# johndpope/SPEAK-hack

Hardware: AMD Instinct MI355X
Metric: generator frames/sec at 256^2, batch 8/GPU (higher is better)
Workload: dtype f32; 1 GPU; StyleGAN decoder (styleganv1.StyleGenerator) 256^2 forward only, batch 8/GPU, fp32, random-init weights, synthetic [8,6144] latents, device-drawn noise; global_batch=8, resolution=256, parallelism=replicas x1 (no data-path collective), launch=hipGraph replay of the step

## Files before the change

### speak-hack_amd/csrc/conv3x3_wino_f32.hip

```cpp
#include "conv_mfma_f32.hpp"

namespace spkwino {

using spkconv::f32x16;
using spkconv::lds_f32_t;
using spkconv::static_for;
typedef float f32x2 __attribute__((ext_vector_type(2)));
typedef float f32x4 __attribute__((ext_vector_type(4)));
typedef __attribute__((address_space(3))) f32x2 lds_f32x2_t;
typedef __attribute__((address_space(3))) f32x2 __attribute__((aligned(4))) lds_f32x2u_t;

constexpr int CO_T = 64, CI_T = 8, NTILE = 64, NT = 256;
constexpr int WIDE = 0, SQUARE = 1;
constexpr int region_w(int shape) { return shape == SQUARE ? 16 : 32; }
constexpr int region_h(int shape) { return shape == SQUARE ? 16 : 8; }
constexpr int RAW_PLANE = 352, RAW_WAVE = 2 * RAW_PLANE;
constexpr int RAW_GATHERS = RAW_WAVE / 64;
constexpr int U_FLOATS = 16 * CI_T * CO_T, V_FLOATS = 16 * CI_T * NTILE, RAW_FLOATS = 4 * RAW_WAVE;
constexpr int U_OFF = 0, V_OFF = 2 * U_FLOATS, RAW_OFF = V_OFF + 2 * V_FLOATS;
constexpr int PRM_OFF = RAW_OFF + 2 * RAW_FLOATS;
constexpr int DEM_OFF = PRM_OFF + 4 * CO_T;
constexpr int RGBW_OFF = DEM_OFF + CO_T;
constexpr int LDS_FLOATS = RGBW_OFF + 3 * CO_T;
constexpr int LDS_BYTES = LDS_FLOATS * 4;
// ... 48 lines not shown
    long long r = idx / CO_T;
    const int ci_l = (int)(r % CI_T);
    r /= CI_T;
    const int xi = (int)(r % 16);
    r /= 16;
    const int chunk = (int)(r % n_chunks), co_tile = (int)(r / n_chunks);
    const int co = co_tile * CO_T + co_l, ci = chunk * CI_T + ci_l;
    float v = 0.f;
    if (co < opCout && ci < opCin) {
        float g[3][3];
#pragma unroll
        for (int a = 0; a < 3; ++a)
#pragma unroll
            for (int b = 0; b < 3; ++b)
                g[a][b] = transpose_flip ? w[(((size_t)ci * Cin + co) * 3 + (2 - a)) * 3 + (2 - b)] : w[(((size_t)co * Cin + ci) * 3 + a) * 3 + b];
        const int i = xi >> 2, j = xi & 3;
        float t[3];
#pragma unroll
        for (int b = 0; b < 3; ++b)
            t[b] = i == 0 ? g[0][b] : (i == 3 ? g[2][b] : 0.5f * ((g[0][b] + g[2][b]) + (i == 1 ? g[1][b] : -g[1][b])));
        v = j == 0 ? t[0] : (j == 3 ? t[2] : 0.5f * ((t[0] + t[2]) + (j == 1 ? t[1] : -t[1])));
    }
    out[idx] = v;
}

struct PackWinoList {
    const float* w[SPK_WINO_PACK_MAX];
    float* out[SPK_WINO_PACK_MAX];
    int Cin[SPK_WINO_PACK_MAX], Cout[SPK_WINO_PACK_MAX], tf[SPK_WINO_PACK_MAX];
};

__global__ void pack_wino_list_kernel(const PackWinoList a) {
    const int it = blockIdx.y;
    const float* __restrict__ w = a.w[it];
    float* __restrict__ out = a.out[it];
    const int Cin = a.Cin[it], Cout = a.Cout[it], transpose_flip = a.tf[it];
    const int opCin = transpose_flip ? Cout : Cin, opCout = transpose_flip ? Cin : Cout;
    const int n_chunks = (opCin + CI_T - 1) / CI_T;
    const long long total = (long long)((opCout + CO_T - 1) / CO_T) * n_chunks * U_FLOATS;
    for (long long idx = (long long)blockIdx.x * blockDim.x + threadIdx.x; idx < total; idx += (long long)gridDim.x * blockDim.x) {
        const int co_l = (int)(idx % CO_T);
        long long r = idx / CO_T;
        const int ci_l = (int)(r % CI_T);
        r /= CI_T;
        const int xi = (int)(r % 16);
        r /= 16;
        const int chunk = (int)(r % n_chunks), co_tile = (int)(r / n_chunks);
        const int co = co_tile * CO_T + co_l, ci = chunk * CI_T + ci_l;
        float v = 0.f;
        if (co < opCout && ci < opCin) {
            float g[3][3];
#pragma unroll
            for (int p = 0; p < 3; ++p)
#pragma unroll
                for (int q = 0; q < 3; ++q)
                    g[p][q] = transpose_flip ? w[(((size_t)ci * Cin + co) * 3 + (2 - p)) * 3 + (2 - q)] : w[(((size_t)co * Cin + ci) * 3 + p) * 3 + q];
            const int i = xi >> 2, j = xi & 3;
            float t[3];
#pragma unroll
            for (int q = 0; q < 3; ++q)
                t[q] = i == 0 ? g[0][q] : (i == 3 ? g[2][q] : 0.5f * ((g[0][q] + g[2][q]) + (i == 1 ? g[1][q] : -g[1][q])));
            v = j == 0 ? t[0] : (j == 3 ? t[2] : 0.5f * ((t[0] + t[2]) + (j == 1 ? t[1] : -t[1])));
        }
        out[idx] = v;
    }
}

__device__ __forceinline__ float fadd_(float a, float b) { float r; asm("v_add_f32 %0, %1, %2" : "=v"(r) : "v"(a), "v"(b)); return r; }
__device__ __forceinline__ float fsub_(float a, float b) { float r; asm("v_sub_f32 %0, %1, %2" : "=v"(r) : "v"(a), "v"(b)); return r; }

__device__ __forceinline__ void up1d_(float a, float b, float c, float nkl, float nkr, float six, float& o0, float& o1, float& o2, float& o3) {
    float e, s, hl, hr;
    asm("v_sub_f32 %0, %9, %7\n\tv_add_f32 %1, %7, %9\n\tv_fma_f32 %2, %8, %12, %1\n\tv_fma_f32 %3, %8, %10, %1\n\t"
        "v_fma_f32 %4, %8, %11, %1\n\tv_fma_f32 %5, %0, -2.0, %3\n\tv_fma_f32 %6, %0, -2.0, -%4"
        : "=&v"(e), "=&v"(s), "=&v"(o1), "=&v"(hl), "=&v"(hr), "=&v"(o0), "=v"(o3)
        : "v"(a), "v"(b), "v"(c), "v"(nkl), "v"(nkr), "s"(six));
    o2 = e;
}

__device__ __forceinline__ void lds_barrier() {
    asm volatile("s_waitcnt lgkmcnt(0)\n\ts_barrier" ::: "memory");
}

template <bool MOD, int SHAPE, bool RGB = false, bool UP = false>
__global__ __launch_bounds__(NT) void wino_kernel(const Args p) {
    static_assert(!(UP && MOD), "the modulated conv keeps its x2 pass");
    constexpr int RW = region_w(SHAPE), RH = region_h(SHAPE), TXN = RW / 2, TYN = RH / 2;
    constexpr int RAW_W = UP ? RW / 2 + 2 : RW + 2, RAW_H = UP ? RH / 2 + 2 : RH + 2, RAW_USED = RAW_W * RAW_H;
    constexpr int PLANE = UP ? UP_PLANE : RAW_PLANE, NG = UP ? UP_GATHERS : RAW_GATHERS;
    extern __shared__ __attribute__((aligned(16))) float smem[];
    const int tid = threadIdx.x, lane = tid & 63;
    const int wave = __builtin_amdgcn_readfirstlane(tid >> 6);
    const int half = lane >> 5, l32 = lane & 31;
    const int wm = wave >> 1, wn = wave & 1;

    const int n_regions = p.regions_x * p.regions_y * p.B * p.ksplit;
    const int xcd = (int)blockIdx.x & 7, wk = (int)blockIdx.x >> 3, wpx = (int)gridDim.x >> 3;
    const int share_q = n_regions >> 3, share_r = n_regions & 7;
    const int reg_begin = xcd * share_q + min(xcd, share_r), reg_end = reg_begin + share_q + (xcd < share_r ? 1 : 0);
    const int grp = (int)blockIdx.y / p.co_tiles_g, co_tile = (int)blockIdx.y - grp * p.co_tiles_g, co0 = co_tile * CO_T;
    const size_t HW = (size_t)p.H * p.W;
    const int Win = UP ? p.W >> 1 : p.W;
    const size_t HWin = UP ? HW >> 2 : HW;

    const __amdgpu_buffer_rsrc_t rsrc = __builtin_amdgcn_make_buffer_rsrc(const_cast<float*>(p.x), 0, (int)p.x_bytes, 0x00020000);
    unsigned voff[NG], voff_next[NG];
    auto region_coords = [&](int item, int& b_, int& y0_, int& x0_, int& kb_) {
        const int reg = item / p.ksplit;
        kb_ = (item - reg * p.ksplit) * p.cps;
        const int rx_ = reg % p.regions_x;
        const int t_ = reg / p.regions_x;
        b_ = t_ / p.regions_y;
        y0_ = (t_ - b_ * p.regions_y) * RH;
        x0_ = rx_ * RW;
    };
    unsigned rel[NG], edge[NG];
#pragma unroll
    for (int k = 0; k < NG; ++k) {
        const int e = k * 64 + lane;
        const int j = e >= PLANE ? 1 : 0, q = e - j * PLANE;
        const int r = q / RAW_W, c = q - r * RAW_W;
        rel[k] = ((unsigned)(wave + 4 * j) * (unsigned)HWin + (unsigned)((r - 1) * Win + (c - 1))) * 4u;
        edge[k] = (r == 0 ? 1u : 0u) | (r == RAW_H - 1 ? 2u : 0u) | (c == 0 ? 4u : 0u) | (c == RAW_W - 1 ? 8u : 0u) | (q >= RAW_USED ? 16u : 0u);
    }
    auto set_voff = [&](unsigned (&vo)[NG], int b_, int y0_, int x0_) {
        const unsigned origin = (((unsigned)b_ * (unsigned)p.Cx + (unsigned)(grp * p.gin)) * (unsigned)HWin +
                                 (unsigned)(UP ? (y0_ >> 1) * Win + (x0_ >> 1) : y0_ * p.W + x0_)) * 4u;
        const unsigned at = (y0_ == 0 ? 1u : 0u) | (y0_ + RH >= p.H ? 2u : 0u) | (x0_ == 0 ? 4u : 0u) | (x0_ + RW >= p.W ? 8u : 0u) | 16u;
        if constexpr (UP) {
            const unsigned row_bytes = (unsigned)Win * 4u;
#pragma unroll
            for (int k = 0; k < NG; ++k) {
                const unsigned h = edge[k] & at;
                vo[k] = (h & 16u) ? 0x80000000u
                                  : origin + rel[k] + ((h & 1u) ? row_bytes : 0u) - ((h & 2u) ? row_bytes : 0u) + ((h & 4u) ? 4u : 0u) - ((h & 8u) ? 4u : 0u);
            }
        } else {
#pragma unroll
            for (int k = 0; k < NG; ++k) vo[k] = (edge[k] & at) ? 0x80000000u : origin + rel[k];
        }
    };
    const unsigned chunk_bytes = (unsigned)(CI_T * HWin * 4);
    const float* wsrc = p.wp + (size_t)blockIdx.y * p.n_chunks * U_FLOATS;

#define WINO_DMA_RAW(vo_in_, chunk_, slot_, k_)                                                                         \
    {                                   \
        const unsigned m0_ = (unsigned)((RAW_OFF + (slot_) * RAW_FLOATS + (k_) * 64) * 4) + raw_m0, vo_ = (vo_in_);     \
        const unsigned so_ = (unsigned)(chunk_) * chunk_bytes;                                                          \
        const __amdgpu_buffer_rsrc_t rs_ = rsrc;                                                                        \
        asm volatile("s_mov_b32 m0, %0\n\ts_nop 0\n\tbuffer_load_dword %1, %2, %3 offen lds" :: "s"(m0_), "v"(vo_), "s"(rs_), "s"(so_)); \
    }
#define WINO_DMA_U(chunk_, slot_, k_)                                                                                   \
    {                                                                                                                   \
        const unsigned m0_ = (unsigned)((U_OFF + (slot_) * U_FLOATS) * 4 + (k_) * 1024) + u_m0, vo_ = lane16;           \
        const float* sb_ = wsrc + (size_t)(chunk_) * U_FLOATS + (wave * U_DMA + (k_)) * 256;                            \
        asm volatile("s_mov_b32 m0, %0\n\ts_nop 0\n\tglobal_load_lds_dwordx4 %1, %2" :: "s"(m0_), "v"(vo_), "s"(sb_));   \
    }
#define WINO_DMA_U_BARE(chunk_, slot_, k_)                                                          \
    {                                                                                                                   \
        const unsigned m0_ = (unsigned)((U_OFF + (slot_) * U_FLOATS) * 4) + u_m0, vo_ = lane16;                         \
        const float* sb_ = wsrc + (size_t)(chunk_) * U_FLOATS + (wave * U_DMA) * 256;                                   \
        if constexpr ((k_) == 0) asm volatile("s_mov_b32 m0, %0\n\ts_nop 0" :: "s"(m0_));                               \
        asm volatile("global_load_lds_dwordx4 %0, %1" :: "v"(vo_), "s"(sb_));                                           \
    }
    const unsigned raw_m0 = (unsigned)(wave * RAW_WAVE * 4), u_m0 = (unsigned)(wave * U_DMA * 1024), lane16 = (unsigned)lane * 16u;

    int a_base = U_OFF + half * CO_T + wm * 32 + l32;
    int b_base = V_OFF + half * NTILE + wn * 32 + l32;
    const int ty_l = lane / TXN, tx_l = lane % TXN;
    int raw_rd = (RAW_OFF + wave * RAW_WAVE + 2 * ty_l * RAW_W + 2 * tx_l) >> 1;
    int v_wr = V_OFF + wave * NTILE + lane;
    asm volatile("" : "+v"(a_base), "+v"(b_base), "+v"(raw_rd), "+v"(v_wr));
    int raw_u[2][2];
    float nk[4] = {-2.f, -2.f, -2.f, -2.f}, nkn[4] = {-2.f, -2.f, -2.f, -2.f};
    const float six = 6.f;
    auto set_nk = [&](float (&k_)[4], int y0_, int x0_) {
        k_[0] = (y0_ == 0 && ty_l == 0) ? -6.f : -2.f;
        k_[1] = (y0_ + RH >= p.H && ty_l == TYN - 1) ? -6.f : -2.f;
        k_[2] = (x0_ == 0 && tx_l == 0) ? -6.f : -2.f;
        k_[3] = (x0_ + RW >= p.W && tx_l == TXN - 1) ? -6.f : -2.f;
    };
    if constexpr (UP) {
#pragma unroll
        for (int rs = 0; rs < 2; ++rs)
#pragma unroll
            for (int j = 0; j < 2; ++j) {
                raw_u[rs][j] = RAW_OFF + wave * RAW_WAVE + ty_l * RAW_W + tx_l + rs * RAW_FLOATS + j * PLANE;
                asm volatile("" : "+v"(raw_u[rs][j]));
            }
    }

    f32x16 acc[16];
    f32x16 zero16;
#pragma unroll
    for (int r = 0; r < 16; ++r) zero16[r] = 0.f;

    float d[2][16], tq[2][16], tv[2][16];
#define WINO_T_READ(rs_, j_, r_)                                                                                        \
    {                                                                                                                   \
        const f32x2 lo_ = *((const volatile lds_f32x2_t*)0 + (raw_rd + ((rs_) * RAW_FLOATS + (j_) * RAW_PLANE + (r_) * RAW_W) / 2)); \
        const f32x2 hi_ = *((const volatile lds_f32x2_t*)0 + (raw_rd + ((rs_) * RAW_FLOATS + (j_) * RAW_PLANE + (r_) * RAW_W + 2) / 2)); \
        d[j_][4 * (r_) + 0] = lo_.x; d[j_][4 * (r_) + 1] = lo_.y; d[j_][4 * (r_) + 2] = hi_.x; d[j_][4 * (r_) + 3] = hi_.y; \
    }
#define WINO_T_ROWS(j_, c_)                                                                                             \
    {                                                                                                                   \
        tq[j_][c_] = fsub_(d[j_][c_], d[j_][8 + (c_)]); tq[j_][4 + (c_)] = fadd_(d[j_][4 + (c_)], d[j_][8 + (c_)]);     \
        tq[j_][8 + (c_)] = fsub_(d[j_][8 + (c_)], d[j_][4 + (c_)]); tq[j_][12 + (c_)] = fsub_(d[j_][4 + (c_)], d[j_][12 + (c_)]); \
    }
#define WINO_T_SCALE(j_, i_, sc_)                                                                                       \
    { tv[j_][4 * (i_)] *= (sc_); tv[j_][4 * (i_) + 1] *= (sc_); tv[j_][4 * (i_) + 2] *= (sc_); tv[j_][4 * (i_) + 3] *= (sc_); }
#define WINO_T_COLS(j_, i_)                                                                                             \
    {                                                                                                                   \
        tv[j_][4 * (i_)] = fsub_(tq[j_][4 * (i_)], tq[j_][4 * (i_) + 2]); tv[j_][4 * (i_) + 1] = fadd_(tq[j_][4 * (i_) + 1], tq[j_][4 * (i_) + 2]); \
        tv[j_][4 * (i_) + 2] = fsub_(tq[j_][4 * (i_) + 2], tq[j_][4 * (i_) + 1]); tv[j_][4 * (i_) + 3] = fsub_(tq[j_][4 * (i_) + 1], tq[j_][4 * (i_) + 3]); \
    }
#define WINO_U_READ(rs_, j_, r_)                                                                                        \
    {                                                                                                                   \
        const volatile lds_f32_t* q_ = (const volatile lds_f32_t*)0 + (raw_u[rs_][j_] + (r_) * RAW_W);                  \
        const f32x2 lo_ = *reinterpret_cast<const volatile lds_f32x2u_t*>(q_);                                          \
        d[j_][3 * (r_) + 0] = lo_.x; d[j_][3 * (r_) + 1] = lo_.y; d[j_][3 * (r_) + 2] = q_[2];                          \
    }
#define WINO_U_H(j_, r_, nk_)                                                                                           \
// ... 22 lines not shown
    b_cur = b;
    kb_cur = kb;
    set_voff(voff, b, y0, x0);
    if constexpr (UP) set_nk(nk, y0, x0);
    static_for<0, U_DMA>([&](auto k) { WINO_DMA_U(kb, 0, decltype(k)::value); });
    static_for<0, NG>([&](auto k) { WINO_DMA_RAW(voff[decltype(k)::value], kb, 0, decltype(k)::value); });
    static_for<0, NG>([&](auto k) { WINO_DMA_RAW(voff[decltype(k)::value], kb + 1, 1, decltype(k)::value); });
    __builtin_amdgcn_s_waitcnt(0x0f70);
    static_for<0, 2>([&](auto j) {
        if constexpr (UP) {
            static_for<0, 3>([&](auto r) { WINO_U_READ(0, decltype(j)::value, decltype(r)::value); });
            static_for<0, 3>([&](auto r) { WINO_U_H(decltype(j)::value, decltype(r)::value, nk); });
            static_for<0, 4>([&](auto c) { WINO_U_V(decltype(j)::value, decltype(c)::value, nk); });
        } else {
            static_for<0, 4>([&](auto r) { WINO_T_READ(0, decltype(j)::value, decltype(r)::value); });
            static_for<0, 4>([&](auto c) { WINO_T_ROWS(decltype(j)::value, decltype(c)::value); });
            static_for<0, 4>([&](auto i) { WINO_T_COLS(decltype(j)::value, decltype(i)::value); });
        }
        if constexpr (MOD) {
            const float sc0_ = p.in_scale[(size_t)b * p.Cin + kb * CI_T + wave + 4 * decltype(j)::value];
            static_for<0, 4>([&](auto i) { WINO_T_SCALE(decltype(j)::value, decltype(i)::value, sc0_); });
        }
        static_for<0, 16>([&](auto xi) { WINO_T_WRITE(0, decltype(j)::value, decltype(xi)::value); });
        __builtin_amdgcn_sched_barrier(0);
    });
    __syncthreads();

#ifndef SPK_WINO_PD
#define SPK_WINO_PD 4
#endif
    constexpr int PD = SPK_WINO_PD;
    float fa[PD + 1], fb[PD + 1];
#define WINO_FRAG(slot_, s_, reg_)                                                                                      \
    {                                                                                                                   \
        constexpr int kk_ = (s_) >> 4, xi_ = (s_) & 15;                                                                 \
        fa[reg_] = *((const volatile lds_f32_t*)0 + (a_base + ((slot_) * U_FLOATS + (xi_ * CI_T + 2 * kk_) * CO_T)));   \
        fb[reg_] = *((const volatile lds_f32_t*)0 + (b_base + ((slot_) * V_FLOATS + (xi_ * CI_T + 2 * kk_) * NTILE)));  \
    }
    auto chunk_body = [&](auto slot_c, auto first_c, const int i, const float (&nk_)[4]) __attribute__((always_inline)) {
        constexpr int S = decltype(slot_c)::value, O = 1 - S;
        constexpr bool FIRST = decltype(first_c)::value;
        const int c1 = i + 1 < n ? kb_cur + i + 1 : kb;
        const int c2 = i + 2 >= n ? kb + i + 2 - n : kb_cur + i + 2;
        float msc[2] = {1.f, 1.f};
        if constexpr (MOD) {
            const float* ms_ = p.in_scale + (size_t)(i + 1 < n ? b_cur : b) * p.Cin + c1 * CI_T + wave;
            msc[0] = ms_[0];
            msc[1] = ms_[4];
        }
        static_for<0, PD>([&](auto s) { WINO_FRAG(S, decltype(s)::value, decltype(s)::value); });
        static_for<0, 64>([&](auto s_c) {
            constexpr int s = decltype(s_c)::value;
            if constexpr (s + PD < 64) { WINO_FRAG(S, s + PD, (s + PD) % (PD + 1)); }
            if constexpr (FIRST && s < 16) acc[s & 15] = __builtin_amdgcn_mfma_f32_32x32x2f32(fa[s % (PD + 1)], fb[s % (PD + 1)], zero16, 0, 0, 0);
            else acc[s & 15] = __builtin_amdgcn_mfma_f32_32x32x2f32(fa[s % (PD + 1)], fb[s % (PD + 1)], acc[s & 15], 0, 0, 0);
            if constexpr (s < U_DMA) {
                if constexpr (KO_UBARE) { WINO_DMA_U_BARE(c1, O, s); }
                else if constexpr (!KO_U) { WINO_DMA_U(c1, O, s); }
            } else if constexpr (s < U_DMA + NG && !KO_RAW) { WINO_DMA_RAW(voff[s - U_DMA], c2, S, s - U_DMA); }
            static_for<0, 2>([&](auto j_c) {
                constexpr int j = decltype(j_c)::value, tr = 2 + 10 * j, ta = 8 + 16 * j;
                if constexpr (UP) {
                    if constexpr (s >= tr && s < tr + 3) { WINO_U_READ(O, j, s - tr); }
                    if constexpr (!KO_TVALU && s >= ta && s < ta + 3) { WINO_U_H(j, s - ta, nk_); }
                    if constexpr (!KO_TVALU && s >= ta + 4 && s < ta + 8) { WINO_U_V(j, s - ta - 4, nk_); }
                } else {
                if constexpr (s >= tr && s < tr + 4) { WINO_T_READ(O, j, s - tr); }
                if constexpr (!KO_TVALU && s >= ta && s < ta + 4) { WINO_T_ROWS(j, s - ta); }
                if constexpr (!KO_TVALU && s >= ta + 4 && s < ta + 8) { WINO_T_COLS(j, s - ta - 4); if constexpr (MOD) { WINO_T_SCALE(j, s - ta - 4, msc[j]); } }
                }
                if constexpr (s >= ta + 8 && s < ta + 16) { WINO_T_WRITE_LOOP(O, j, 2 * (s - ta - 8)); WINO_T_WRITE_LOOP(O, j, 2 * (s - ta - 8) + 1); }
            });
            __builtin_amdgcn_sched_barrier(0);
        });
        __builtin_amdgcn_s_waitcnt(0x0f70);
        __syncthreads();
    };
    const bool f_bias = p.flags & SPK_EPI_BIAS, f_noise = p.flags & SPK_EPI_NOISE;
    const bool f_lrelu = p.flags & SPK_EPI_LRELU, f_style = p.flags & SPK_EPI_STYLE, f_accum = p.flags & SPK_EPI_ACCUM;
    const float osc = p.out_scale_dev ? p.out_scale * *p.out_scale_dev : p.out_scale;
    const float slope_ = f_lrelu ? p.slope : 1.f, gain_ = f_lrelu ? p.act_gain : 1.f;
    const int tile = wn * 32 + l32, oy = 2 * (tile / TXN), ox = 2 * (tile % TXN);
    const int row_lane = wm * 32 + 4 * half;
    const int prm_which = tid & 3, prm_c = co0 + (tid >> 2);
    const bool prm_on = prm_c < p.Cout && (prm_which == 0 ? f_bias : (prm_which == 1 ? f_noise : f_style));
    const float* const prm_src = (prm_which == 0 ? p.bias : (prm_which == 1 ? p.noise_w : p.style + (prm_which == 3 ? p.Cout : 0))) + prm_c;
    const float prm_neutral = prm_which == 2 ? 1.f : 0.f;

    using F_ = std::false_type;
#ifdef SPK_WINO_LAB
    unsigned long long lab_t[8] = {0, 0, 0, 0, 0, 0, 0, 0};
    int lab_region = 0;
#define LAB_STAMP(k_) { if (lab_region == 1) lab_t[k_] = __builtin_readcyclecounter(); }
#else
#define LAB_STAMP(k_)
#endif
    for (;;) {
        LAB_STAMP(0)
#pragma unroll
        for (int xi = 0; xi < 16; ++xi)
#pragma unroll
            for (int r = 0; r < 16; ++r) acc[xi][r] = 0.f;
        const int cur_b = b, cur_y0 = y0, cur_x0 = x0;
        b_cur = b;
        kb_cur = kb;
        const size_t pix = (size_t)(cur_y0 + oy) * p.W + (cur_x0 + ox);
        f32x2 nz0, nz1;
        nz0.x = nz0.y = nz1.x = nz1.y = 0.f;
        if (f_noise) {
            nz0 = *reinterpret_cast<const f32x2*>(p.noise + (size_t)cur_b * HW + pix);
            nz1 = *reinterpret_cast<const f32x2*>(p.noise + (size_t)cur_b * HW + pix + p.W);
        }
        float prm = prm_neutral;
        if (prm_on) {
            const float t_ = prm_src[prm_which >= 2 ? (size_t)cur_b * p.style_stride : 0];
            prm = prm_which == 2 ? t_ + 1.f : t_;
        }
        float dem = 1.f;
        if constexpr (MOD) {
            if (p.out_scale_bc && tid < CO_T && co0 + tid < p.Cout) dem = p.out_scale_bc[(size_t)cur_b * p.Cout + co0 + tid];
        }
        const bool more = reg + wpx < reg_end;
        if (more) {
            reg += wpx;
            region_coords(reg, b, y0, x0, kb);
        }
        set_voff(voff_next, b, y0, x0);
        if constexpr (UP) {
            set_nk(nk, cur_y0, cur_x0);
            set_nk(nkn, y0, x0);
        }

        LAB_STAMP(1)
        for (int i = 0; i < n; i += 2) {
            const bool last_pair = i + 2 >= n;
            if constexpr (UP) {
#pragma unroll
                for (int k = 0; k < NG; ++k) voff[k] = last_pair ? voff_next[k] : voff[k];
            } else if (last_pair) {
                asm volatile("" ::: "memory");
#pragma unroll
                for (int k = 0; k < NG; ++k) voff[k] = voff_next[k];
            }
            chunk_body(std::integral_constant<int, 0>{}, F_{}, i, nk);
            if constexpr (UP) {
                float nk2[4];
#pragma unroll
                for (int k = 0; k < 4; ++k) nk2[k] = last_pair ? nkn[k] : nk[k];
                chunk_body(std::integral_constant<int, 1>{}, F_{}, i + 1, nk2);
            } else {
                chunk_body(std::integral_constant<int, 1>{}, F_{}, i + 1, nk);
            }
        }

        LAB_STAMP(2)
        smem[PRM_OFF + tid] = prm;
        if constexpr (MOD) { if (tid < CO_T) smem[DEM_OFF + tid] = dem; }
        lds_barrier();
        unsigned hw_ = (unsigned)HW;
        asm volatile("" : "+s"(hw_));
        const size_t o0 = ((size_t)cur_b * p.Cy + (size_t)grp * p.Cout) * hw_ + pix + (size_t)(kb_cur / p.cps) * p.slice_floats;
        LAB_STAMP(3)
#define WINO_ACC(xi_, r_) ({ float v_; asm volatile("v_accvgpr_read_b32 %0, %1" : "=v"(v_) : "a"(acc[xi_][r_])); v_; })
        float rgb[3][4];
#pragma unroll
        for (int o = 0; o < 3; ++o)
#pragma unroll
            for (int q = 0; q < 4; ++q) rgb[o][q] = 0.f;
        static_for<0, 16>([&](auto r_c) {
            constexpr int r = decltype(r_c)::value;
            const int row = row_lane + (r & 3) + 8 * (r >> 2);
            const float4 q_ = *reinterpret_cast<const float4*>(smem + PRM_OFF + 4 * row);
            float s0[4], s1[4];
#pragma unroll
            for (int i = 0; i < 4; ++i) {
                const float m0 = WINO_ACC(4 * i, r), m1 = WINO_ACC(4 * i + 1, r), m2 = WINO_ACC(4 * i + 2, r), m3 = WINO_ACC(4 * i + 3, r);
                s0[i] = (m0 + m1) + m2;
                s1[i] = (m1 - m2) - m3;
            }
            f32x2 top, bot;
            top.x = (s0[0] + s0[1]) + s0[2]; top.y = (s1[0] + s1[1]) + s1[2];
            bot.x = (s0[1] - s0[2]) - s0[3]; bot.y = (s1[1] - s1[2]) - s1[3];
            float osc_r = osc;
            if constexpr (MOD) osc_r = osc * smem[DEM_OFF + row];
            top.x = top.x * osc_r + q_.x; top.y = top.y * osc_r + q_.x; bot.x = bot.x * osc_r + q_.x; bot.y = bot.y * osc_r + q_.x;
            top.x += q_.y * nz0.x; top.y += q_.y * nz0.y; bot.x += q_.y * nz1.x; bot.y += q_.y * nz1.y;
            top.x = (top.x > 0.f ? top.x : top.x * slope_) * gain_; top.y = (top.y > 0.f ? top.y : top.y * slope_) * gain_;
            bot.x = (bot.x > 0.f ? bot.x : bot.x * slope_) * gain_; bot.y = (bot.y > 0.f ? bot.y : bot.y * slope_) * gain_;
            const int co = co0 + row;
            if constexpr (RGB) {
                top.x = top.x * q_.z + q_.w; top.y = top.y * q_.z + q_.w; bot.x = bot.x * q_.z + q_.w; bot.y = bot.y * q_.z + q_.w;
#pragma unroll
                for (int o = 0; o < 3; ++o) {
                    const float w_ = smem[RGBW_OFF + o * CO_T + row];
                    rgb[o][0] += w_ * top.x; rgb[o][1] += w_ * top.y; rgb[o][2] += w_ * bot.x; rgb[o][3] += w_ * bot.y;
                }
                if (p.y && co < p.Cout) {
                    const size_t off = o0 + (size_t)co * hw_;
                    *reinterpret_cast<f32x2*>(p.y + off) = top;
                    *reinterpret_cast<f32x2*>(p.y + off + p.W) = bot;
                }
                __builtin_amdgcn_sched_barrier(0);
            } else if (co < p.Cout) {
                const size_t off = o0 + (size_t)co * hw_;
                if (p.y_pre) {
                    *reinterpret_cast<f32x2*>(p.y_pre + off) = top;
                    *reinterpret_cast<f32x2*>(p.y_pre + off + p.W) = bot;
                }
                top.x = top.x * q_.z + q_.w; top.y = top.y * q_.z + q_.w; bot.x = bot.x * q_.z + q_.w; bot.y = bot.y * q_.z + q_.w;
                if (f_accum) {
                    const f32x2 o_t = *reinterpret_cast<const f32x2*>(p.y + off), o_b = *reinterpret_cast<const f32x2*>(p.y + off + p.W);
                    top.x += o_t.x; top.y += o_t.y; bot.x += o_b.x; bot.y += o_b.y;
                }
#ifdef SPK_WINO_NOSTORE
                if (top.x == 12345.678f)
#endif
                {
                    *reinterpret_cast<f32x2*>(p.y + off) = top;
                    *reinterpret_cast<f32x2*>(p.y + off + p.W) = bot;
                }
            }
        });
#undef WINO_ACC
        if constexpr (RGB) {
            float* part = smem + RGB_PART_OFF + ((wm * 2 + half) * NTILE + tile) * 12;
#pragma unroll
            for (int o = 0; o < 3; ++o) *reinterpret_cast<float4*>(part + 4 * o) = make_float4(rgb[o][0], rgb[o][1], rgb[o][2], rgb[o][3]);
            lds_barrier();
            if (tid < 3 * NTILE) {
                const int o = tid >> 6, t = tid & (NTILE - 1);
                const float* ps = smem + RGB_PART_OFF + t * 12 + 4 * o;
                float4 v = *reinterpret_cast<const float4*>(ps);
#pragma unroll
                for (int g = 1; g < 4; ++g) {
                    const float4 u = *reinterpret_cast<const float4*>(ps + g * NTILE * 12);
                    v.x += u.x; v.y += u.y; v.z += u.z; v.w += u.w;
                }
                const float bo = p.rgb_bias ? p.rgb_bias[o] : 0.f;
                const size_t off = ((size_t)cur_b * 3 + o) * hw_ + (size_t)(cur_y0 + 2 * (t / TXN)) * p.W + (cur_x0 + 2 * (t % TXN));
                f32x2 a_, b_;
                a_.x = v.x + bo; a_.y = v.y + bo; b_.x = v.z + bo; b_.y = v.w + bo;
                *reinterpret_cast<f32x2*>(p.rgb_y + off) = a_;
                *reinterpret_cast<f32x2*>(p.rgb_y + off + p.W) = b_;
            }
        }
        LAB_STAMP(4)
        lds_barrier();
#ifdef SPK_WINO_LAB
        if (lab_region == 1 && blockIdx.x == 8 && blockIdx.y == 0 && tid == 0)
            for (int k = 0; k < 5; ++k) p.y[k] = (float)(long long)(lab_t[k] - lab_t[0]);
        ++lab_region;
#endif
        if (!more) break;
    }
#undef WINO_FRAG
#undef WINO_T_WRITE_LOOP
#undef WINO_T_WRITE
#undef WINO_U_V
#undef WINO_U_H
#undef WINO_U_READ
#undef WINO_T_COLS
#undef WINO_T_SCALE
#undef WINO_T_ROWS
#undef WINO_T_READ
#undef WINO_DMA_U_BARE
#undef WINO_DMA_U
#undef WINO_DMA_RAW
}

}

using namespace spkwino;

extern "C" {

int64_t spk_conv2d_packed_bytes_wino(int Cin, int Cout) {
    if (Cin <= 0 || Cout <= 0) return -1;
    return (int64_t)spk::ceil_div(Cout, CO_T) * spk::ceil_div(Cin, CI_T) * U_FLOATS * 4;
}

int spk_conv2d_pack_weights_wino(const float* w, float* w_packed, int Cin, int Cout, int transpose_flip, void* stream) {
    SPK_REQUIRE(w && w_packed && Cin > 0 && Cout > 0 && (transpose_flip == 0 || transpose_flip == 1), "pack_weights_wino: bad arguments");
    const int opCin = transpose_flip ? Cout : Cin, opCout = transpose_flip ? Cin : Cout;
    const int n_chunks = spk::ceil_div(opCin, CI_T);
    const long long total = (long long)spk::ceil_div(opCout, CO_T) * n_chunks * U_FLOATS;
    hipLaunchKernelGGL(pack_wino_kernel, dim3((unsigned)((total + 255) / 256)), dim3(256), 0, (hipStream_t)stream, w, w_packed, Cin, Cout,
                       opCin, opCout, transpose_flip, n_chunks, total);
    return spk::check_launch("pack_wino_kernel");
}

static int wino_shape(int H, int W) {
    if (H % region_h(WIDE) == 0 && W % region_w(WIDE) == 0) return WIDE;
    if (H % region_h(SQUARE) == 0 && W % region_w(SQUARE) == 0) return SQUARE;
    return -1;
}

int spk_conv2d_pack_weights_wino_list(const float* const* w, float* const* w_packed, const int* Cin, const int* Cout, const int* transpose_flip,
                                      int n, void* stream) {
    SPK_REQUIRE(w && w_packed && Cin && Cout && transpose_flip && n > 0 && n <= SPK_WINO_PACK_MAX, "pack_weights_wino_list: 1..%d items", SPK_WINO_PACK_MAX);
    PackWinoList a;
    long long most = 0;
    for (int i = 0; i < n; ++i) {
        SPK_REQUIRE(w[i] && w_packed[i] && Cin[i] > 0 && Cout[i] > 0 && (transpose_flip[i] == 0 || transpose_flip[i] == 1), "pack_weights_wino_list: item %d", i);
        a.w[i] = w[i]; a.out[i] = w_packed[i]; a.Cin[i] = Cin[i]; a.Cout[i] = Cout[i]; a.tf[i] = transpose_flip[i];
        most = std::max<long long>(most, (transpose_flip[i] ? spk_conv2d_packed_bytes_wino(Cout[i], Cin[i]) : spk_conv2d_packed_bytes_wino(Cin[i], Cout[i])) / 4);
    }
    dim3 grid((unsigned)std::min<long long>((most + 255) / 256, 2048), (unsigned)n);
    hipLaunchKernelGGL(pack_wino_list_kernel, grid, dim3(256), 0, (hipStream_t)stream, a);
    return spk::check_launch("pack_wino_list_kernel");
}

static int wino_geometry_ok(int B, int Cin, int Cout, int H, int W) {
    if (B <= 0 || Cin <= 0 || Cout <= 0 || H <= 0 || W <= 0) return 0;
    if (wino_shape(H, W) < 0) return 0;
    if (Cin % (2 * CI_T)) return 0;
    return 1;
}

int spk_conv2d_wino_supported(int B, int Cin, int Cout, int H, int W) {
    if (!wino_geometry_ok(B, Cin, Cout, H, W)) return 0;
    if ((long long)B * Cin * H * W * 4 >= (1ll << 31)) return 0;
    return 1;
}

int spk_conv2d_wino_up_supported(int B, int Cin, int Cout, int H, int W) {
    if (!wino_geometry_ok(B, Cin, Cout, H, W) || (H & 1) || (W & 1)) return 0;
    if ((long long)B * Cin * (H / 2) * (W / 2) * 4 >= (1ll << 31)) return 0;
    return 1;
}

int spk_conv2d_wino_ksplit(int want, int B, int Cin, int Cout, int H, int W) {
    if (!wino_geometry_ok(B, Cin, Cout, H, W)) return -1;
    const int shape = wino_shape(H, W), n_chunks = Cin / CI_T;
    const long long pairs = (long long)B * (H / region_h(shape)) * (W / region_w(shape)) * spk::ceil_div(Cout, CO_T);
    auto ok = [&](int ks) { return ks >= 1 && n_chunks % (2 * ks) == 0 && n_chunks / ks >= 4; };
    if (want > 0) {
        int ks = want;
        while (ks > 1 && !ok(ks)) --ks;
        return ks;
    }
    int ks = 1;
    while (pairs * ks < 192 && ok(2 * ks)) ks *= 2;
    return ks;
}

int64_t spk_conv2d_wino_workspace_bytes(int ksplit, int B, int Cin, int Cout, int H, int W) {
    const int ks = spk_conv2d_wino_ksplit(ksplit, B, Cin, Cout, H, W);
    if (ks < 0) return -1;
    return ks > 1 ? (int64_t)ks * B * Cout * H * W * 4 : 0;
}

int spk_conv2d_wino_fwd(const spk_conv2d_desc* d, void* stream) {
    SPK_REQUIRE(d && d->x && d->w_packed, "conv2d winograd: null pointer");
    SPK_REQUIRE(d->kh == 3 && d->kw == 3 && d->stride == 1, "conv2d winograd: 3x3 stride-1 kernels only");
    const int G = d->groups > 1 ? d->groups : 1;
    const bool up = d->flags & SPK_CONV_UPSAMPLE2X;
    SPK_REQUIRE(!up || (G == 1 && !(d->flags & (SPK_CONV_IN_BATCH_SCALE | SPK_CONV_UP_FIR1331))),
                "conv2d winograd: SPK_CONV_UPSAMPLE2X is the bilinear x2 of a plain launch (no IN_BATCH_SCALE, no UP_FIR1331, no groups): "
                "pass the x2 image (spk_upsample2x_fwd)");
    SPK_REQUIRE(G == 1 || !(d->flags & ~(SPK_CONV_WINOGRAD | SPK_EPI_ACCUM)), "conv2d winograd: a grouped launch takes SPK_EPI_ACCUM only (the encoders' "
                "data gradients)");
    const int gin = G > 1 ? d->group_in_stride : d->Cin, Cx = gin * (G - 1) + d->Cin, Cy = G * d->Cout;
    SPK_REQUIRE(G == 1 || gin >= d->Cin, "conv2d winograd: groups read disjoint channels");
    const unsigned epi = SPK_EPI_BIAS | SPK_EPI_NOISE | SPK_EPI_LRELU | SPK_EPI_STYLE | SPK_EPI_ACCUM;
    const unsigned allowed = SPK_CONV_WINOGRAD | epi | SPK_CONV_IN_BATCH_SCALE | SPK_EPI_TORGB | SPK_CONV_UPSAMPLE2X;
    SPK_REQUIRE(!(d->flags & ~allowed) && !d->stats && !d->accum_half,
                "conv2d winograd: plain, bilinear x2 or batch-scaled input; epilogue flags bias, noise, lrelu, style, accum, torgb");
    const bool mod = d->flags & SPK_CONV_IN_BATCH_SCALE, rgb = d->flags & SPK_EPI_TORGB;
    SPK_REQUIRE(d->y || rgb, "conv2d winograd: null pointer");
    if (rgb)
        SPK_REQUIRE(d->rgb_w && d->rgb_y && d->rgb_channels == 3 && d->Cout <= CO_T && !mod && !d->y_pre && !(d->flags & SPK_EPI_ACCUM) &&
                        (reinterpret_cast<uintptr_t>(d->rgb_y) & 7) == 0,
                    "conv2d winograd: SPK_EPI_TORGB needs rgb_w [3][Cout], rgb_y [B,3,H,W], Cout <= 64 (one channel tile), no y_pre / accumulate / modulation");
    SPK_REQUIRE(!mod || d->in_scale, "conv2d winograd: IN_BATCH_SCALE without in_scale[B,Cin]");
    SPK_REQUIRE(!d->out_scale_bc || mod, "conv2d winograd: out_scale_bc (demodulation) goes with SPK_CONV_IN_BATCH_SCALE");
    if (up)
        SPK_REQUIRE(d->H == 2 * d->Hin && d->W == 2 * d->Win && spk_conv2d_wino_up_supported(d->B, d->Cin, d->Cout, d->H, d->W),
                    "conv2d winograd: SPK_CONV_UPSAMPLE2X needs an output of twice the input size, %dx%d -> %dx%d", d->Hin, d->Win, d->H, d->W);
    else
        SPK_REQUIRE(d->H == d->Hin && d->W == d->Win, "conv2d winograd: output size must equal the input size");
    SPK_REQUIRE(wino_geometry_ok(d->B, d->Cin, d->Cout, d->H, d->W) && (long long)d->B * Cx * d->Hin * d->Win * 4 < (1ll << 31),
                "conv2d winograd: %dx%d is not a whole number of 32 x 8 or 16 x 16 regions (or the input exceeds 2 GB)", d->H, d->W);
    SPK_REQUIRE(!(d->flags & SPK_EPI_BIAS) || d->bias, "conv2d winograd: SPK_EPI_BIAS without bias");
    SPK_REQUIRE(!(d->flags & SPK_EPI_NOISE) || (d->noise && d->noise_w), "conv2d winograd: SPK_EPI_NOISE without noise");
    SPK_REQUIRE(!(d->flags & SPK_EPI_STYLE) || d->style, "conv2d winograd: SPK_EPI_STYLE without style");
    const auto aligned16 = [](const void* q) { return (reinterpret_cast<uintptr_t>(q) & 15) == 0; };
    SPK_REQUIRE(aligned16(d->w_packed) && aligned16(d->y) && aligned16(d->y_pre) && aligned16(d->noise) && (reinterpret_cast<uintptr_t>(d->x) & 3) == 0,
                "conv2d winograd: tensors must be 16-byte aligned");
    const int shape = wino_shape(d->H, d->W);
    const int ks = spk_conv2d_wino_ksplit(d->ksplit, d->B, d->Cin, Cy, d->H, d->W);
    const size_t out_floats = (size_t)d->B * Cy * d->H * d->W;
    if (ks > 1)
        SPK_REQUIRE(d->workspace && aligned16(d->workspace) && d->workspace_bytes >= (int64_t)ks * (int64_t)out_floats * 4,
                    "conv2d winograd: %d contraction slices need a workspace of %lld bytes (spk_conv2d_wino_workspace_bytes)", ks,
                    (long long)ks * (long long)out_floats * 4);
    Args a;
    a.x = d->x; a.wp = d->w_packed; a.bias = d->bias; a.noise_w = d->noise_w; a.noise = d->noise; a.style = d->style;
    a.y = d->y; a.y_pre = d->y_pre; a.out_scale_dev = d->out_scale_dev;
    a.in_scale = mod ? d->in_scale : nullptr; a.out_scale_bc = d->out_scale_bc;
    a.rgb_w = d->rgb_w; a.rgb_bias = d->rgb_bias; a.rgb_y = d->rgb_y;
    a.B = d->B; a.Cin = d->Cin; a.Cout = d->Cout; a.H = d->H; a.W = d->W;
    a.G = G; a.gin = gin; a.Cx = Cx; a.Cy = Cy; a.co_tiles_g = spk::ceil_div(d->Cout, CO_T);
    a.regions_x = d->W / region_w(shape); a.regions_y = d->H / region_h(shape);
    a.n_chunks = spk::ceil_div(d->Cin, CI_T);
    a.ksplit = ks; a.cps = a.n_chunks / ks; a.slice_floats = 0;
    a.style_stride = d->style_stride; a.flags = d->flags;
    a.x_bytes = (unsigned)((long long)d->B * Cx * d->Hin * d->Win * 4);
    const float up_scale = up ? 0.0625f : 1.f;
    a.slope = d->lrelu_slope; a.out_scale = d->out_scale * up_scale; a.act_gain = d->act_gain != 0.f ? d->act_gain : 1.f;
    SPK_REQUIRE(!rgb || ks == 1, "conv2d winograd: SPK_EPI_TORGB with a sliced contraction (%d slices): pass ksplit = 1 or run the 1x1 separately", ks);
    if (ks > 1) {
        a.y = static_cast<float*>(d->workspace); a.y_pre = nullptr; a.out_scale_dev = nullptr; a.out_scale_bc = nullptr;
        a.flags = d->flags & ~epi; a.out_scale = 1.f; a.slice_floats = out_floats;
    }
    spkconv::ConvArgs f = {};
    if (ks > 1) {
        f.bias = d->bias; f.noise_w = d->noise_w; f.noise = d->noise; f.style = d->style; f.out_scale_bc = d->out_scale_bc;
        f.y = d->y; f.y_pre = d->y_pre; f.B = d->B; f.Cin = d->Cin; f.Cout = d->Cout; f.Cy = Cy; f.Cx = Cx; f.G = G; f.H = d->H; f.W = d->W;
        f.style_stride = d->style_stride; f.flags = d->flags & epi; f.slope = d->lrelu_slope; f.out_scale = d->out_scale * up_scale;
        f.act_gain = a.act_gain; f.out_scale_dev = d->out_scale_dev;
    }
    if (spkconv::form_probe) return spkconv::report_sliced_form(f, static_cast<const float*>(d->workspace), ks);
    void (*kern)(const Args) = mod ? (shape == SQUARE ? &wino_kernel<true, SQUARE> : &wino_kernel<true, WIDE>)
                               : rgb ? (shape == SQUARE ? &wino_kernel<false, SQUARE, true> : &wino_kernel<false, WIDE, true>)
                                     : (shape == SQUARE ? &wino_kernel<false, SQUARE> : &wino_kernel<false, WIDE>);
    if (up)
        kern = rgb ? (shape == SQUARE ? &wino_kernel<false, SQUARE, true, true> : &wino_kernel<false, WIDE, true, true>)
                   : (shape == SQUARE ? &wino_kernel<false, SQUARE, false, true> : &wino_kernel<false, WIDE, false, true>);
    static bool raised[10] = {false, false, false, false, false, false, false, false, false, false};
    const int which = (mod ? 2 : rgb ? 4 : 0) + (shape == SQUARE ? 1 : 0) + (up ? (rgb ? 4 : 6) : 0);
    if (!raised[which]) {
        hipError_t e = hipFuncSetAttribute(reinterpret_cast<const void*>(kern), hipFuncAttributeMaxDynamicSharedMemorySize, 160 * 1024);
        if (e != hipSuccess) return spk::fail(SPK_ELAUNCH, "hipFuncSetAttribute(LDS): %s", hipGetErrorString(e));
        raised[which] = true;
    }
    const long long n_items = (long long)a.regions_x * a.regions_y * d->B * ks;
    SPK_REQUIRE(n_items < (1ll << 31), "conv2d winograd: grid too large");
    const int co_tiles = G * spk::ceil_div(d->Cout, CO_T);
    static int n_cu = 0;
    if (n_cu == 0) {
        int dev = 0;
        hipDeviceProp_t prop;
        if (hipGetDevice(&dev) != hipSuccess || hipGetDeviceProperties(&prop, dev) != hipSuccess) return spk::fail(SPK_ELAUNCH, "conv2d winograd: no device properties");
        n_cu = prop.multiProcessorCount > 0 ? prop.multiProcessorCount : 256;
    }
    long long gx = std::max(8ll, ((long long)n_cu / co_tiles) / 8 * 8);
    static int lab_mult = -1;
    if (lab_mult < 0) { const char* e = getenv("SPK_WINO_WGS"); lab_mult = e ? atoi(e) : 1; }
    gx = lab_mult == 0 ? (n_items + 7) / 8 * 8 : gx * lab_mult;
    gx = std::min(gx, (n_items + 7) / 8 * 8);
    dim3 grid((unsigned)gx, (unsigned)co_tiles);
    hipLaunchKernelGGL(kern, grid, dim3(NT), LDS_BYTES, (hipStream_t)stream, a);
    int rc = spk::check_launch("wino_kernel");
    if (rc != SPK_OK || ks == 1) return rc;
    return spkconv::launch_splitk_epilogue(f, static_cast<const float*>(d->workspace), ks, (hipStream_t)stream);
}

}
```

Baseline: 4094 frames/s.

## Add lean epilogue variants to Winograd conv and pack edge masks

Adds an EPI template parameter that selects a lean epilogue when the call has no y_pre, no accumulation, no modulation and a positive leaky-ReLU slope. The lean form uses fmax for leaky ReLU, drops the per-row channel bounds checks, and uses precomputed row base pointers. When a fused toRGB call has no activation output it skips the activation store entirely. The output transform is rewritten as inline asm that reads the accumulators directly, edge flags are bit-packed into fewer registers, and parameter-load setup moves into the loop, all aimed at lower register pressure and epilogue instruction count. The cost is more kernel instantiations and stricter applicability conditions.

```diff
diff --git a/speak-hack_amd/csrc/conv3x3_wino_f32.hip b/speak-hack_amd/csrc/conv3x3_wino_f32.hip
--- a/speak-hack_amd/csrc/conv3x3_wino_f32.hip
+++ b/speak-hack_amd/csrc/conv3x3_wino_f32.hip
@@ -154,9 +154,12 @@
     asm volatile("s_waitcnt lgkmcnt(0)\n\ts_barrier" ::: "memory");
 }
 
-template <bool MOD, int SHAPE, bool RGB = false, bool UP = false>
+constexpr int GENERIC = 0, LEAN = 1, LEAN_NOSTORE = 2;
+template <bool MOD, int SHAPE, bool RGB = false, bool UP = false, int EPI = GENERIC>
 __global__ __launch_bounds__(NT) void wino_kernel(const Args p) {
     static_assert(!(UP && MOD), "the modulated conv keeps its x2 pass");
+    static_assert(EPI == GENERIC || !MOD, "the modulated forms keep the generic rows");
+    static_assert(EPI != LEAN_NOSTORE || RGB, "only a fused toRGB launch may leave the activation unwritten");
     constexpr int RW = region_w(SHAPE), RH = region_h(SHAPE), TXN = RW / 2, TYN = RH / 2;
     constexpr int RAW_W = UP ? RW / 2 + 2 : RW + 2, RAW_H = UP ? RH / 2 + 2 : RH + 2, RAW_USED = RAW_W * RAW_H;
     constexpr int PLANE = UP ? UP_PLANE : RAW_PLANE, NG = UP ? UP_GATHERS : RAW_GATHERS;
@@ -186,14 +189,18 @@
         y0_ = (t_ - b_ * p.regions_y) * RH;
         x0_ = rx_ * RW;
     };
-    unsigned rel[NG], edge[NG];
+    constexpr int NE = (NG + 5) / 6;
+    unsigned rel[NG], edges[NE];
+#pragma unroll
+    for (int k = 0; k < NE; ++k) edges[k] = 0u;
+#define WINO_EDGE(k_) ((edges[(k_) / 6] >> (5 * ((k_) % 6))) & 31u)
 #pragma unroll
     for (int k = 0; k < NG; ++k) {
         const int e = k * 64 + lane;
         const int j = e >= PLANE ? 1 : 0, q = e - j * PLANE;
         const int r = q / RAW_W, c = q - r * RAW_W;
         rel[k] = ((unsigned)(wave + 4 * j) * (unsigned)HWin + (unsigned)((r - 1) * Win + (c - 1))) * 4u;
-        edge[k] = (r == 0 ? 1u : 0u) | (r == RAW_H - 1 ? 2u : 0u) | (c == 0 ? 4u : 0u) | (c == RAW_W - 1 ? 8u : 0u) | (q >= RAW_USED ? 16u : 0u);
+        edges[k / 6] |= ((r == 0 ? 1u : 0u) | (r == RAW_H - 1 ? 2u : 0u) | (c == 0 ? 4u : 0u) | (c == RAW_W - 1 ? 8u : 0u) | (q >= RAW_USED ? 16u : 0u)) << (5 * (k % 6));
     }
     auto set_voff = [&](unsigned (&vo)[NG], int b_, int y0_, int x0_) {
         const unsigned origin = (((unsigned)b_ * (unsigned)p.Cx + (unsigned)(grp * p.gin)) * (unsigned)HWin +
@@ -203,13 +210,13 @@
             const unsigned row_bytes = (unsigned)Win * 4u;
 #pragma unroll
             for (int k = 0; k < NG; ++k) {
-                const unsigned h = edge[k] & at;
+                const unsigned h = WINO_EDGE(k) & at;
                 vo[k] = (h & 16u) ? 0x80000000u
                                   : origin + rel[k] + ((h & 1u) ? row_bytes : 0u) - ((h & 2u) ? row_bytes : 0u) + ((h & 4u) ? 4u : 0u) - ((h & 8u) ? 4u : 0u);
             }
         } else {
 #pragma unroll
-            for (int k = 0; k < NG; ++k) vo[k] = (edge[k] & at) ? 0x80000000u : origin + rel[k];
+            for (int k = 0; k < NG; ++k) vo[k] = (WINO_EDGE(k) & at) ? 0x80000000u : origin + rel[k];
         }
     };
     const unsigned chunk_bytes = (unsigned)(CI_T * HWin * 4);
@@ -398,10 +405,8 @@
     const float slope_ = f_lrelu ? p.slope : 1.f, gain_ = f_lrelu ? p.act_gain : 1.f;
     const int tile = wn * 32 + l32, oy = 2 * (tile / TXN), ox = 2 * (tile % TXN);
     const int row_lane = wm * 32 + 4 * half;
-    const int prm_which = tid & 3, prm_c = co0 + (tid >> 2);
-    const bool prm_on = prm_c < p.Cout && (prm_which == 0 ? f_bias : (prm_which == 1 ? f_noise : f_style));
-    const float* const prm_src = (prm_which == 0 ? p.bias : (prm_which == 1 ? p.noise_w : p.style + (prm_which == 3 ? p.Cout : 0))) + prm_c;
-    const float prm_neutral = prm_which == 2 ? 1.f : 0.f;
+    float rgb_bo = 0.f;
+    if constexpr (RGB) { if (p.rgb_bias) rgb_bo = p.rgb_bias[min(wave, 2)]; }
 
     using F_ = std::false_type;
 #ifdef SPK_WINO_LAB
@@ -427,11 +432,13 @@
             nz0 = *reinterpret_cast<const f32x2*>(p.noise + (size_t)cur_b * HW + pix);
             nz1 = *reinterpret_cast<const f32x2*>(p.noise + (size_t)cur_b * HW + pix + p.W);
         }
-        float prm = prm_neutral;
-        if (prm_on) {
-            const float t_ = prm_src[prm_which >= 2 ? (size_t)cur_b * p.style_stride : 0];
-            prm = prm_which == 2 ? t_ + 1.f : t_;
-        }
+        int prm_t = tid;
+        asm volatile("" : "+v"(prm_t));
+        const int prm_which = prm_t & 3, prm_c = co0 + (prm_t >> 2);
+        const bool prm_on = prm_c < p.Cout && (prm_which == 0 ? f_bias : (prm_which == 1 ? f_noise : f_style));
+        const float* const prm_src = (prm_which == 0 ? p.bias : (prm_which == 1 ? p.noise_w : p.style + (prm_which == 3 ? p.Cout : 0))) + prm_c;
+        float prm_raw = 0.f;
+        if (prm_on) prm_raw = prm_src[prm_which >= 2 ? (size_t)cur_b * p.style_stride : 0];
         float dem = 1.f;
         if constexpr (MOD) {
             if (p.out_scale_bc && tid < CO_T && co0 + tid < p.Cout) dem = p.out_scale_bc[(size_t)cur_b * p.Cout + co0 + tid];
@@ -470,14 +477,36 @@
         }
 
         LAB_STAMP(2)
-        smem[PRM_OFF + tid] = prm;
+        smem[PRM_OFF + tid] = (tid & 3) == 2 ? prm_raw + 1.f : prm_raw;
         if constexpr (MOD) { if (tid < CO_T) smem[DEM_OFF + tid] = dem; }
         lds_barrier();
         unsigned hw_ = (unsigned)HW;
         asm volatile("" : "+s"(hw_));
         const size_t o0 = ((size_t)cur_b * p.Cy + (size_t)grp * p.Cout) * hw_ + pix + (size_t)(kb_cur / p.cps) * p.slice_floats;
+        const size_t hw_bytes = (size_t)hw_ * 4, w_bytes = (size_t)p.W * 4;
+        char* const y_rows = reinterpret_cast<char*>(p.y + ((size_t)cur_b * p.Cy + (size_t)grp * p.Cout + co0 + wm * 32) * hw_ +
+                                                     (size_t)(kb_cur / p.cps) * p.slice_floats);
+        const unsigned y_lane = ((unsigned)(4 * half) * hw_ + (unsigned)pix) * 4u;
         LAB_STAMP(3)
-#define WINO_ACC(xi_, r_) ({ float v_; asm volatile("v_accvgpr_read_b32 %0, %1" : "=v"(v_) : "a"(acc[xi_][r_])); v_; })
+#define WINO_ROW4(a_, b_, m0_, m1_, m2_, m3_)                                                                           \
+    "v_accvgpr_read_b32 " a_ ", " m0_ "\n\tv_accvgpr_read_b32 " b_ ", " m1_ "\n\tv_accvgpr_read_b32 %4, " m2_ "\n\tv_accvgpr_read_b32 %5, " m3_ "\n\t" \
+    "v_add_f32 " a_ ", " a_ ", " b_ "\n\tv_sub_f32 " b_ ", " b_ ", %4\n\tv_add_f32 " a_ ", " a_ ", %4\n\tv_sub_f32 " b_ ", " b_ ", %5\n\t"
+#define WINO_ROW(r_, top_, bot_)                                                                                        \
+    {                                                                                                                   \
+        float tx_, ty_, bx_, by_, t0_, t1_, t2_, t3_;                                                                   \
+        asm volatile(WINO_ROW4("%0", "%1", "%8", "%9", "%10", "%11")                                                    \
+                     WINO_ROW4("%2", "%3", "%12", "%13", "%14", "%15")                                                  \
+                     "v_add_f32 %0, %0, %2\n\tv_add_f32 %1, %1, %3\n\t"                                                \
+                     WINO_ROW4("%6", "%7", "%16", "%17", "%18", "%19")                                                  \
+                     "v_add_f32 %0, %0, %6\n\tv_sub_f32 %2, %2, %6\n\tv_add_f32 %1, %1, %7\n\tv_sub_f32 %3, %3, %7\n\t" \
+                     WINO_ROW4("%6", "%7", "%20", "%21", "%22", "%23")                                                  \
+                     "v_sub_f32 %2, %2, %6\n\tv_sub_f32 %3, %3, %7"                                                    \
+                     : "=&v"(tx_), "=&v"(ty_), "=&v"(bx_), "=&v"(by_), "=&v"(t0_), "=&v"(t1_), "=&v"(t2_), "=&v"(t3_)    \
+                     : "a"(acc[0][r_]), "a"(acc[1][r_]), "a"(acc[2][r_]), "a"(acc[3][r_]), "a"(acc[4][r_]), "a"(acc[5][r_]), \
+                       "a"(acc[6][r_]), "a"(acc[7][r_]), "a"(acc[8][r_]), "a"(acc[9][r_]), "a"(acc[10][r_]), "a"(acc[11][r_]), \
+                       "a"(acc[12][r_]), "a"(acc[13][r_]), "a"(acc[14][r_]), "a"(acc[15][r_]));                         \
+        (top_).x = tx_; (top_).y = ty_; (bot_).x = bx_; (bot_).y = by_;                                                 \
+    }
         float rgb[3][4];
 #pragma unroll
         for (int o = 0; o < 3; ++o)
@@ -487,64 +516,81 @@
             constexpr int r = decltype(r_c)::value;
             const int row = row_lane + (r & 3) + 8 * (r >> 2);
             const float4 q_ = *reinterpret_cast<const float4*>(smem + PRM_OFF + 4 * row);
-            float s0[4], s1[4];
-#pragma unroll
-            for (int i = 0; i < 4; ++i) {
-                const float m0 = WINO_ACC(4 * i, r), m1 = WINO_ACC(4 * i + 1, r), m2 = WINO_ACC(4 * i + 2, r), m3 = WINO_ACC(4 * i + 3, r);
-                s0[i] = (m0 + m1) + m2;
-                s1[i] = (m1 - m2) - m3;
-            }
             f32x2 top, bot;
-            top.x = (s0[0] + s0[1]) + s0[2]; top.y = (s1[0] + s1[1]) + s1[2];
-            bot.x = (s0[1] - s0[2]) - s0[3]; bot.y = (s1[1] - s1[2]) - s1[3];
+            WINO_ROW(r, top, bot)
             float osc_r = osc;
             if constexpr (MOD) osc_r = osc * smem[DEM_OFF + row];
             top.x = top.x * osc_r + q_.x; top.y = top.y * osc_r + q_.x; bot.x = bot.x * osc_r + q_.x; bot.y = bot.y * osc_r + q_.x;
             top.x += q_.y * nz0.x; top.y += q_.y * nz0.y; bot.x += q_.y * nz1.x; bot.y += q_.y * nz1.y;
-            top.x = (top.x > 0.f ? top.x : top.x * slope_) * gain_; top.y = (top.y > 0.f ? top.y : top.y * slope_) * gain_;
-            bot.x = (bot.x > 0.f ? bot.x : bot.x * slope_) * gain_; bot.y = (bot.y > 0.f ? bot.y : bot.y * slope_) * gain_;
-            const int co = co0 + row;
-            if constexpr (RGB) {
+            if constexpr (EPI != GENERIC) {
+                top.x = __builtin_fmaxf(top.x, top.x * slope_) * gain_; top.y = __builtin_fmaxf(top.y, top.y * slope_) * gain_;
+                bot.x = __builtin_fmaxf(bot.x, bot.x * slope_) * gain_; bot.y = __builtin_fmaxf(bot.y, bot.y * slope_) * gain_;
                 top.x = top.x * q_.z + q_.w; top.y = top.y * q_.z + q_.w; bot.x = bot.x * q_.z + q_.w; bot.y = bot.y * q_.z + q_.w;
-#pragma unroll
-                for (int o = 0; o < 3; ++o) {
-                    const float w_ = smem[RGBW_OFF + o * CO_T + row];
-                    rgb[o][0] += w_ * top.x; rgb[o][1] += w_ * top.y; rgb[o][2] += w_ * bot.x; rgb[o][3] += w_ * bot.y;
+                if constexpr (RGB) {
+#pragma unroll
+                    for (int o = 0; o < 3; ++o) {
+                        const float w_ = smem[RGBW_OFF + o * CO_T + row];
+                        rgb[o][0] += w_ * top.x; rgb[o][1] += w_ * top.y; rgb[o][2] += w_ * bot.x; rgb[o][3] += w_ * bot.y;
+                    }
                 }
-                if (p.y && co < p.Cout) {
+                if constexpr (EPI == LEAN) {
+                    char* const yr = y_rows + (size_t)((r & 3) + 8 * (r >> 2)) * hw_bytes;
+#ifdef SPK_WINO_NOSTORE
+                    if (top.x == 12345.678f)
+#endif
+                    {
+                        *reinterpret_cast<f32x2*>(yr + y_lane) = top;
+                        *reinterpret_cast<f32x2*>(yr + w_bytes + y_lane) = bot;
+                    }
+                }
+                if constexpr (RGB) __builtin_amdgcn_sched_barrier(0);
+            } else {
+                top.x = (top.x > 0.f ? top.x : top.x * slope_) * gain_; top.y = (top.y > 0.f ? top.y : top.y * slope_) * gain_;
+                bot.x = (bot.x > 0.f ? bot.x : bot.x * slope_) * gain_; bot.y = (bot.y > 0.f ? bot.y : bot.y * slope_) * gain_;
+                const int co = co0 + row;
+                if constexpr (RGB) {
+                    top.x = top.x * q_.z + q_.w; top.y = top.y * q_.z + q_.w; bot.x = bot.x * q_.z + q_.w; bot.y = bot.y * q_.z + q_.w;
+#pragma unroll
+                    for (int o = 0; o < 3; ++o) {
+                        const float w_ = smem[RGBW_OFF + o * CO_T + row];
+                        rgb[o][0] += w_ * top.x; rgb[o][1] += w_ * top.y; rgb[o][2] += w_ * bot.x; rgb[o][3] += w_ * bot.y;
+                    }
+                    if (p.y && co < p.Cout) {
+                        char* const yr = y_rows + (size_t)((r & 3) + 8 * (r >> 2)) * hw_bytes;
+                        *reinterpret_cast<f32x2*>(yr + y_lane) = top;
+                        *reinterpret_cast<f32x2*>(yr + w_bytes + y_lane) = bot;
+                    }
+                    __builtin_amdgcn_sched_barrier(0);
+                } else if (co < p.Cout) {
                     const size_t off = o0 + (size_t)co * hw_;
-                    *reinterpret_cast<f32x2*>(p.y + off) = top;
-                    *reinterpret_cast<f32x2*>(p.y + off + p.W) = bot;
-                }
-                __builtin_amdgcn_sched_barrier(0);
-            } else if (co < p.Cout) {
-                const size_t off = o0 + (size_t)co * hw_;
-                if (p.y_pre) {
-                    *reinterpret_cast<f32x2*>(p.y_pre + off) = top;
-                    *reinterpret_cast<f32x2*>(p.y_pre + off + p.W) = bot;
-                }
-                top.x = top.x * q_.z + q_.w; top.y = top.y * q_.z + q_.w; bot.x = bot.x * q_.z + q_.w; bot.y = bot.y * q_.z + q_.w;
-                if (f_accum) {
-                    const f32x2 o_t = *reinterpret_cast<const f32x2*>(p.y + off), o_b = *reinterpret_cast<const f32x2*>(p.y + off + p.W);
-                    top.x += o_t.x; top.y += o_t.y; bot.x += o_b.x; bot.y += o_b.y;
-                }
+                    if (p.y_pre) {
+                        *reinterpret_cast<f32x2*>(p.y_pre + off) = top;
+                        *reinterpret_cast<f32x2*>(p.y_pre + off + p.W) = bot;
+                    }
+                    top.x = top.x * q_.z + q_.w; top.y = top.y * q_.z + q_.w; bot.x = bot.x * q_.z + q_.w; bot.y = bot.y * q_.z + q_.w;
+                    if (f_accum) {
+                        const f32x2 o_t = *reinterpret_cast<const f32x2*>(p.y + off), o_b = *reinterpret_cast<const f32x2*>(p.y + off + p.W);
+                        top.x += o_t.x; top.y += o_t.y; bot.x += o_b.x; bot.y += o_b.y;
+                    }
 #ifdef SPK_WINO_NOSTORE
-                if (top.x == 12345.678f)
+                    if (top.x == 12345.678f)
 #endif
-                {
-                    *reinterpret_cast<f32x2*>(p.y + off) = top;
-                    *reinterpret_cast<f32x2*>(p.y + off + p.W) = bot;
+                    {
+                        *reinterpret_cast<f32x2*>(p.y + off) = top;
+                        *reinterpret_cast<f32x2*>(p.y + off + p.W) = bot;
+                    }
                 }
             }
         });
-#undef WINO_ACC
+#undef WINO_ROW
+#undef WINO_ROW4
         if constexpr (RGB) {
             float* part = smem + RGB_PART_OFF + ((wm * 2 + half) * NTILE + tile) * 12;
 #pragma unroll
             for (int o = 0; o < 3; ++o) *reinterpret_cast<float4*>(part + 4 * o) = make_float4(rgb[o][0], rgb[o][1], rgb[o][2], rgb[o][3]);
             lds_barrier();
-            if (tid < 3 * NTILE) {
-                const int o = tid >> 6, t = tid & (NTILE - 1);
+            {
+                const int o = min(wave, 2), t = lane;
                 const float* ps = smem + RGB_PART_OFF + t * 12 + 4 * o;
                 float4 v = *reinterpret_cast<const float4*>(ps);
 #pragma unroll
@@ -552,12 +598,12 @@
                     const float4 u = *reinterpret_cast<const float4*>(ps + g * NTILE * 12);
                     v.x += u.x; v.y += u.y; v.z += u.z; v.w += u.w;
                 }
-                const float bo = p.rgb_bias ? p.rgb_bias[o] : 0.f;
-                const size_t off = ((size_t)cur_b * 3 + o) * hw_ + (size_t)(cur_y0 + 2 * (t / TXN)) * p.W + (cur_x0 + 2 * (t % TXN));
+                char* const yo = reinterpret_cast<char*>(p.rgb_y + ((size_t)cur_b * 3 + o) * hw_ + (size_t)cur_y0 * p.W + cur_x0);
+                const unsigned t_off = ((unsigned)(2 * (t / TXN)) * (unsigned)p.W + (unsigned)(2 * (t % TXN))) * 4u;
                 f32x2 a_, b_;
-                a_.x = v.x + bo; a_.y = v.y + bo; b_.x = v.z + bo; b_.y = v.w + bo;
-                *reinterpret_cast<f32x2*>(p.rgb_y + off) = a_;
-                *reinterpret_cast<f32x2*>(p.rgb_y + off + p.W) = b_;
+                a_.x = v.x + rgb_bo; a_.y = v.y + rgb_bo; b_.x = v.z + rgb_bo; b_.y = v.w + rgb_bo;
+                *reinterpret_cast<f32x2*>(yo + t_off) = a_;
+                *reinterpret_cast<f32x2*>(yo + (size_t)p.W * 4 + t_off) = b_;
             }
         }
         LAB_STAMP(4)
@@ -582,6 +628,7 @@
 #undef WINO_DMA_U_BARE
 #undef WINO_DMA_U
 #undef WINO_DMA_RAW
+#undef WINO_EDGE
 }
 
 }
@@ -737,18 +784,29 @@
         f.act_gain = a.act_gain; f.out_scale_dev = d->out_scale_dev;
     }
     if (spkconv::form_probe) return spkconv::report_sliced_form(f, static_cast<const float*>(d->workspace), ks);
+    const bool lrelu_ok = !(a.flags & SPK_EPI_LRELU) || (a.slope > 0.f && a.slope <= 1.f);
+    const bool lean_ok = !mod && lrelu_ok && !a.y_pre && !(a.flags & SPK_EPI_ACCUM) && 20ll * d->H * d->W < (1ll << 32);
+    const int epi_form = !lean_ok ? GENERIC : rgb ? (!a.y ? LEAN_NOSTORE : d->Cout == CO_T ? LEAN : GENERIC) : (d->Cout % CO_T == 0 ? LEAN : GENERIC);
+    const auto pick = [&](auto rgb_c, auto up_c) -> void (*)(const Args) {
+        constexpr bool R = decltype(rgb_c)::value, U = decltype(up_c)::value;
+        if constexpr (R) {
+            if (epi_form == LEAN_NOSTORE) return shape == SQUARE ? &wino_kernel<false, SQUARE, R, U, LEAN_NOSTORE> : &wino_kernel<false, WIDE, R, U, LEAN_NOSTORE>;
+        }
+        if (epi_form == LEAN) return shape == SQUARE ? &wino_kernel<false, SQUARE, R, U, LEAN> : &wino_kernel<false, WIDE, R, U, LEAN>;
+        return shape == SQUARE ? &wino_kernel<false, SQUARE, R, U> : &wino_kernel<false, WIDE, R, U>;
+    };
+    using T_ = std::true_type;
+    using F_ = std::false_type;
     void (*kern)(const Args) = mod ? (shape == SQUARE ? &wino_kernel<true, SQUARE> : &wino_kernel<true, WIDE>)
-                               : rgb ? (shape == SQUARE ? &wino_kernel<false, SQUARE, true> : &wino_kernel<false, WIDE, true>)
-                                     : (shape == SQUARE ? &wino_kernel<false, SQUARE> : &wino_kernel<false, WIDE>);
-    if (up)
-        kern = rgb ? (shape == SQUARE ? &wino_kernel<false, SQUARE, true, true> : &wino_kernel<false, WIDE, true, true>)
-                   : (shape == SQUARE ? &wino_kernel<false, SQUARE, false, true> : &wino_kernel<false, WIDE, false, true>);
-    static bool raised[10] = {false, false, false, false, false, false, false, false, false, false};
-    const int which = (mod ? 2 : rgb ? 4 : 0) + (shape == SQUARE ? 1 : 0) + (up ? (rgb ? 4 : 6) : 0);
-    if (!raised[which]) {
+                               : rgb ? (up ? pick(T_{}, T_{}) : pick(T_{}, F_{})) : (up ? pick(F_{}, T_{}) : pick(F_{}, F_{}));
+    static const void* raised[32];
+    static int n_raised = 0;
+    bool seen = false;
+    for (int i = 0; i < n_raised; ++i) seen = seen || raised[i] == reinterpret_cast<const void*>(kern);
+    if (!seen) {
         hipError_t e = hipFuncSetAttribute(reinterpret_cast<const void*>(kern), hipFuncAttributeMaxDynamicSharedMemorySize, 160 * 1024);
         if (e != hipSuccess) return spk::fail(SPK_ELAUNCH, "hipFuncSetAttribute(LDS): %s", hipGetErrorString(e));
-        raised[which] = true;
+        if (n_raised < 32) raised[n_raised++] = reinterpret_cast<const void*>(kern);
     }
     const long long n_items = (long long)a.regions_x * a.regions_y * d->B * ks;
     SPK_REQUIRE(n_items < (1ll << 31), "conv2d winograd: grid too large");
```

Result: faster. 4233 frames/s, median of 6 (+3.4%).
